# Crowsinc/LiveVisionKit

Hardware: AMD Instinct MI355X
Metric: stabilized frames/sec (one 4K YUV420 stream per GPU, steady state) (higher is better)
Workload: dtype f32

## Files before the change

### include/lvk_hip.h

```cpp
#ifndef LVK_HIP_H
#define LVK_HIP_H

#include <stdint.h>
#include <stddef.h>

#ifdef __cplusplus
extern "C" {
#endif

#define LVK_HIP_OK              0
#define LVK_HIP_ERR_ARG        -1
#define LVK_HIP_ERR_RUNTIME    -2
#define LVK_HIP_ERR_NO_DEVICE  -3

typedef struct lvk_hip_ctx lvk_hip_ctx;


int  lvk_hip_ctx_create(int device, lvk_hip_ctx** out);
int  lvk_hip_ctx_create_on_stream(int device, void* hip_stream, lvk_hip_ctx** out);
void lvk_hip_ctx_destroy(lvk_hip_ctx* ctx);
int  lvk_hip_sync(lvk_hip_ctx* ctx);
void* lvk_hip_stream(lvk_hip_ctx* ctx);
const char* lvk_hip_last_error(lvk_hip_ctx* ctx);
const char* lvk_hip_version(void);
// ... 188 lines not shown
int  lvk_hip_fsr_easu(lvk_hip_ctx* ctx, const void* d_src, int src_step, int rows, int cols, int format, const int region_xywh[4], void* d_dst,
                      int dst_step, int out_rows, int out_cols);
int  lvk_hip_fsr_geometry(int rows, int cols, int out_rows, int out_cols, float multiplier, int maintain_aspect_ratio, const int crop_ltrb[4],
                          int region_xywh[4], int out_rows_cols[2], int* skip);
int  lvk_hip_text_size(const char* text, int scale, int thickness, int wh[2], int* baseline);



int  lvk_hip_stab_prefetch(lvk_hip_stab* stab, const void* d_frame, int step, int rows, int cols, int format);
int  lvk_hip_stab_prefetch_yuv420(lvk_hip_stab* stab, const void* d_y, int y_step, const void* d_u, int u_step, const void* d_v, int v_step,
                                  int nv12, int rows, int cols);
long long lvk_hip_stab_lookahead_frames(lvk_hip_stab* stab);

#define LVK_SCHED_PUSH_FREE_RUNNING   0
#define LVK_SCHED_PUSH_SYNCHRONISED   1
#define LVK_SCHED_INGEST_ON_TRACKER   2
#define LVK_SCHED_INGEST_ON_BULK      3
#define LVK_SCHED_INGEST_INLINE       4
#define LVK_SCHED_REMAP_PERSISTENT    5
#define LVK_SCHED_REMAP_FULL          6
#define LVK_SCHED_WAIT_SIGNAL_WORD    7
#define LVK_SCHED_WAIT_EVENT          8
#define LVK_SCHED_WAIT_WORD_TIMEOUT   9
#define LVK_SCHED_COUNT              10
int  lvk_hip_stab_schedule_counters(lvk_hip_stab* stab, long long out[LVK_SCHED_COUNT], int reset);

int  lvk_hip_stab_get_stats(const lvk_hip_stab* stab, lvk_stab_stats* out);
int  lvk_hip_stab_detector_frames(const lvk_hip_stab* stab, long long* on_device, long long* on_host);
int  lvk_hip_stab_get_meshes(const lvk_hip_stab* stab, float* motion, float* correction, int cap_floats);
int  lvk_hip_stab_get_features(const lvk_hip_stab* stab, float* xy_resp_age, int cap);


#define LVK_STAGE_DOWNSCALE 0
#define LVK_STAGE_PYRAMID   1
#define LVK_STAGE_FAST      2
#define LVK_STAGE_PYRLK     3
#define LVK_STAGE_MOTION    4
#define LVK_STAGE_REMAP     5
#define LVK_STAGE_INGEST    6
#define LVK_STAGE_EGRESS    7
#define LVK_STAGE_COUNT     8
int  lvk_hip_stab_set_profiling(lvk_hip_stab* stab, int enable);
int  lvk_hip_stab_get_profile(lvk_hip_stab* stab, double total_ms[LVK_STAGE_COUNT], long long launches[LVK_STAGE_COUNT]);

int lvk_hip_native_rcp(lvk_hip_ctx* ctx, const float* d_in, float* d_out, size_t n);

typedef struct lvk_hip_mesh_solver lvk_hip_mesh_solver;
// ... 64 lines not shown
```

### livevisionkit_amd/csrc/ingest.hip

```cpp
#include "lvk_hip_internal.hpp"

#include <cmath>
#include <algorithm>
#include <string>

#define LVK_STREAM_STORE(ptr, v) __builtin_nontemporal_store((uint32_t)(v), (ptr))

namespace {

__device__ __forceinline__ uint32_t lin8(const uint8_t* __restrict__ r0, const uint8_t* __restrict__ r1, int pix,
                                         const Lin8Entry tx, int b0, int b1)
{
    const int h0 = r0[tx.s0 * pix] * tx.a0 + r0[tx.s1 * pix] * tx.a1;
    const int h1 = r1[tx.s0 * pix] * tx.a0 + r1[tx.s1 * pix] * tx.a1;
    return (uint32_t)((((b0 * (h0 >> 4)) >> 16) + ((b1 * (h1 >> 4)) >> 16) + 2) >> 2) & 0xffu;
}

template <bool NV12>
__global__ __launch_bounds__(256)
void k_ingest_yuv420(const uint8_t* __restrict__ yp, int y_step, const uint8_t* __restrict__ up, int u_step,
                     const uint8_t* __restrict__ vp, int v_step, int rows, int cols,
                     uint8_t* __restrict__ dst, int dst_step, const Lin8Entry* __restrict__ xtab, const Lin8Entry* __restrict__ ytab, int fast)
{
    const int x0 = (blockIdx.x * 64 + threadIdx.x) * 4;
// ... 9 lines not shown
#pragma unroll
    for (int p = 0; p < 4; p++)
    {
        px[p] = 0;
        if (p < npx)
        {
            const Lin8Entry tx = xtab[x0 + p];
            px[p] = (uint32_t)yp[(long)y * y_step + x0 + p] | (lin8(u0, u1, PIX, tx, ty.a0, ty.a1) << 8) | (lin8(v0, v1, PIX, tx, ty.a0, ty.a1) << 16);
        }
    }
    uint8_t* drow = dst + (long)y * dst_step;
    if (fast && npx == 4)
    {
        uint32_t* d = reinterpret_cast<uint32_t*>(drow + 3 * x0);
        d[0] = px[0] | (px[1] << 24);
        d[1] = (px[1] >> 8) | (px[2] << 16);
        d[2] = (px[2] >> 16) | (px[3] << 8);
    }
    else
        for (int p = 0; p < npx; p++) { uint8_t* d = drow + 3 * (x0 + p); d[0] = (uint8_t)px[p]; d[1] = (uint8_t)(px[p] >> 8); d[2] = (uint8_t)(px[p] >> 16); }
}

template <bool NV12>
__global__ __launch_bounds__(256)
void k_ingest_yuv420_x2(const uint8_t* __restrict__ yp, int y_step, const uint8_t* __restrict__ up, int u_step,
                        const uint8_t* __restrict__ vp, int v_step, int rows, int cols, uint8_t* __restrict__ dst, int dst_step)
{
    LVK_TL(0);
    const int x0 = (blockIdx.x * 64 + threadIdx.x) * 4;
    const int k = blockIdx.y * 4 + threadIdx.y;
    const int cc = cols >> 1, cr = rows >> 1;
    if (x0 >= cols || k > cr) return;
    const int r0 = max(k - 1, 0), r1 = min(k, cr - 1);
    const int c0 = x0 >> 1;
    const bool left = x0 == 0, right = x0 == cols - 4;
    const int lc = left ? 0 : (right ? cc - 4 : c0 - 1);
    struct __attribute__((packed, aligned(1))) P4 { uint32_t w; };
    struct __attribute__((packed, aligned(1))) P8 { uint32_t w[2]; };
    uint32_t su0, su1, sv0, sv1;
    if (NV12)
    {
        const P8 a = *reinterpret_cast<const P8*>(up + (long)r0 * u_step + 2 * lc);
        const P8 b = *reinterpret_cast<const P8*>(up + (long)r1 * u_step + 2 * lc);
        su0 = __builtin_amdgcn_perm(a.w[1], a.w[0], 0x06040200u); sv0 = __builtin_amdgcn_perm(a.w[1], a.w[0], 0x07050301u);
        su1 = __builtin_amdgcn_perm(b.w[1], b.w[0], 0x06040200u); sv1 = __builtin_amdgcn_perm(b.w[1], b.w[0], 0x07050301u);
    }
    else
    {
        su0 = reinterpret_cast<const P4*>(up + (long)r0 * u_step + lc)->w;
        su1 = reinterpret_cast<const P4*>(up + (long)r1 * u_step + lc)->w;
        sv0 = reinterpret_cast<const P4*>(vp + (long)r0 * v_step + lc)->w;
// ... 12 lines not shown
    const int ya = 2 * k - 1, yb = 2 * k;
    const bool has_a = ya >= 0, has_b = yb < rows;
    const uint32_t ywa = has_a ? *reinterpret_cast<const uint32_t*>(yp + (long)ya * y_step + x0) : 0u;
    const uint32_t ywb = has_b ? *reinterpret_cast<const uint32_t*>(yp + (long)yb * y_step + x0) : 0u;
    uint32_t pa[4], pb[4];
#pragma unroll
    for (int p = 0; p < 4; p++)
    {
        const uint32_t u0 = tu0[p], u1 = tu1[p], v0 = tv0[p], v1 = tv1[p];
        const uint32_t ua = ((((u0 + u0 + u0) >> 2) + (u1 >> 2) + 2u) >> 2), ub = (((u0 >> 2) + ((u1 + u1 + u1) >> 2) + 2u) >> 2);
        const uint32_t va = ((((v0 + v0 + v0) >> 2) + (v1 >> 2) + 2u) >> 2), vb = (((v0 >> 2) + ((v1 + v1 + v1) >> 2) + 2u) >> 2);
        pa[p] = ((ywa >> (8 * p)) & 0xffu) | (ua << 8) | (va << 16);
        pb[p] = ((ywb >> (8 * p)) & 0xffu) | (ub << 8) | (vb << 16);
    }
    if (has_a)
    {
        uint32_t* d = reinterpret_cast<uint32_t*>(dst + (long)ya * dst_step + 3 * x0);
        LVK_STREAM_STORE(d + 0, pa[0] | (pa[1] << 24)); LVK_STREAM_STORE(d + 1, (pa[1] >> 8) | (pa[2] << 16)); LVK_STREAM_STORE(d + 2, (pa[2] >> 16) | (pa[3] << 8));
    }
    if (has_b)
    {
        uint32_t* d = reinterpret_cast<uint32_t*>(dst + (long)yb * dst_step + 3 * x0);
        LVK_STREAM_STORE(d + 0, pb[0] | (pb[1] << 24)); LVK_STREAM_STORE(d + 1, (pb[1] >> 8) | (pb[2] << 16)); LVK_STREAM_STORE(d + 2, (pb[2] >> 16) | (pb[3] << 8));
    }
}

template <bool NV12>
__global__ __launch_bounds__(256)
void k_egress_yuv420(const uint8_t* __restrict__ src, int src_step, int rows, int cols,
                     uint8_t* __restrict__ yp, int y_step, uint8_t* __restrict__ up, int u_step, uint8_t* __restrict__ vp, int v_step)
{
    const int cx = blockIdx.x * 64 + threadIdx.x;
    const int cy = blockIdx.y * 4 + threadIdx.y;
    if (cx >= cols / 2 || cy >= rows / 2) return;
    const uint8_t* p0 = src + (long)(2 * cy) * src_step + 6 * (long)cx;
    const uint8_t* p1 = p0 + src_step;
    uint8_t a[6], b[6];
#pragma unroll
    for (int i = 0; i < 6; i++) { a[i] = p0[i]; b[i] = p1[i]; }
    uint8_t* y0 = yp + (long)(2 * cy) * y_step + 2 * cx;
    y0[0] = a[0]; y0[1] = a[3]; y0[y_step] = b[0]; y0[y_step + 1] = b[3];
    const uint8_t u = (uint8_t)((a[1] + a[4] + b[1] + b[4] + 2) >> 2);
    const uint8_t v = (uint8_t)((a[2] + a[5] + b[2] + b[5] + 2) >> 2);
    if (NV12) { uint8_t* d = up + (long)cy * u_step + 2 * cx; d[0] = u; d[1] = v; }
    else { up[(long)cy * u_step + cx] = u; vp[(long)cy * v_step + cx] = v; }
}
// ... 271 lines not shown
        {
            e.s0 = std::min(std::max(s, 0), ssize - 1); e.s1 = std::min(std::max(s + 1, 0), ssize - 1);
            e.a0 = (int)lrintf((1.f - f) * 2048.f); e.a1 = (int)lrintf(f * 2048.f);
        }
        else
        {
            if (s < 0) { f = 0.f; s = 0; }
            bool single = false;
            if (s + 1 >= ssize) { single = true; if (s >= ssize - 1) { f = 0.f; s = ssize - 1; } }
            e.s0 = s; e.s1 = single ? s : s + 1;
            e.a0 = single ? 2048 : (int)lrintf((1.f - f) * 2048.f); e.a1 = single ? 0 : (int)lrintf(f * 2048.f);
        }
        tab[(size_t)d] = e;
    }
    Lin8Entry* d_tab = nullptr;
    LVK_HIP_CHECK(ctx, hipMalloc((void**)&d_tab, tab.size() * sizeof(Lin8Entry)));
    LVK_HIP_CHECK(ctx, hipMemcpy(d_tab, tab.data(), tab.size() * sizeof(Lin8Entry), hipMemcpyHostToDevice));
    ctx->lin8tabs[key] = d_tab;
    *d_out = d_tab;
    return LVK_HIP_OK;
}

int lvk_launch_ingest_yuv420(lvk_hip_ctx* ctx, hipStream_t stream, const void* d_y, int y_step, const void* d_u, int u_step,
                             const void* d_v, int v_step, int nv12, int rows, int cols, void* d_dst, int dst_step)
{
    LVK_HIP_REQUIRE(ctx, d_y && d_u && (nv12 || d_v) && d_dst && rows > 0 && cols > 0);
    LVK_HIP_REQUIRE(ctx, (rows & 1) == 0 && (cols & 1) == 0);
    LVK_HIP_REQUIRE(ctx, y_step >= cols && dst_step >= 3 * cols && u_step >= (nv12 ? cols : cols / 2));
    const Lin8Entry *xt, *yt;
    int rc;
    if ((rc = lvk_get_lin8tab(ctx, cols / 2, cols, false, &xt)) != LVK_HIP_OK) return rc;
    if ((rc = lvk_get_lin8tab(ctx, rows / 2, rows, true, &yt)) != LVK_HIP_OK) return rc;
    const int fast = ((reinterpret_cast<uintptr_t>(d_dst) | (uintptr_t)dst_step) & 3u) == 0 ? 1 : 0;
    const dim3 block(64, 4), grid1((cols / 4 + 63 + (cols % 4 ? 1 : 0)) / 64, (rows + 3) / 4);
    const bool x2 = fast && cols % 4 == 0 && cols >= 16 && rows >= 4 &&
                    ((reinterpret_cast<uintptr_t>(d_y) | (uintptr_t)y_step) & 3u) == 0;
    if (x2)
    {
        const dim3 grid(grid1.x, (rows / 2 + 1 + 3) / 4);
        if (nv12) hipLaunchKernelGGL(k_ingest_yuv420_x2<true>, grid, block, 0, stream, (const uint8_t*)d_y, y_step, (const uint8_t*)d_u, u_step,
                                     (const uint8_t*)d_u, u_step, rows, cols, (uint8_t*)d_dst, dst_step);
        else hipLaunchKernelGGL(k_ingest_yuv420_x2<false>, grid, block, 0, stream, (const uint8_t*)d_y, y_step, (const uint8_t*)d_u, u_step,
                                (const uint8_t*)d_v, v_step, rows, cols, (uint8_t*)d_dst, dst_step);
        LVK_HIP_CHECK(ctx, hipGetLastError());
        return LVK_HIP_OK;
    }
    const dim3 grid = grid1;
    if (nv12)
        hipLaunchKernelGGL(k_ingest_yuv420<true>, grid, block, 0, stream, (const uint8_t*)d_y, y_step, (const uint8_t*)d_u, u_step, (const uint8_t*)d_u, u_step,
                           rows, cols, (uint8_t*)d_dst, dst_step, xt, yt, fast);
    else
        hipLaunchKernelGGL(k_ingest_yuv420<false>, grid, block, 0, stream, (const uint8_t*)d_y, y_step, (const uint8_t*)d_u, u_step, (const uint8_t*)d_v, v_step,
                           rows, cols, (uint8_t*)d_dst, dst_step, xt, yt, fast);
    LVK_HIP_CHECK(ctx, hipGetLastError());
    return LVK_HIP_OK;
}

int lvk_launch_egress_yuv420(lvk_hip_ctx* ctx, hipStream_t stream, const void* d_src, int src_step, int rows, int cols,
                             void* d_y, int y_step, void* d_u, int u_step, void* d_v, int v_step, int nv12)
{
    LVK_HIP_REQUIRE(ctx, d_src && d_y && d_u && (nv12 || d_v) && rows > 0 && cols > 0);
    LVK_HIP_REQUIRE(ctx, (rows & 1) == 0 && (cols & 1) == 0);
    LVK_HIP_REQUIRE(ctx, src_step >= 3 * cols && y_step >= cols && u_step >= (nv12 ? cols : cols / 2));
    const dim3 block(64, 4), grid((cols / 2 + 63) / 64, (rows / 2 + 3) / 4);
    if (nv12)
        hipLaunchKernelGGL(k_egress_yuv420<true>, grid, block, 0, stream, (const uint8_t*)d_src, src_step, rows, cols, (uint8_t*)d_y, y_step, (uint8_t*)d_u, u_step, (uint8_t*)d_u, u_step);
    else
// ... 23 lines not shown
        LVK_HIP_REQUIRE(ctx, (cols & 1) == 0 && steps[0] >= 2 * cols);
        return LVK_HIP_OK;
    case LVK_VIDEO_FORMAT_I444: case LVK_VIDEO_FORMAT_YUVA:
        LVK_HIP_REQUIRE(ctx, p1 && p2 && steps[0] >= cols && steps[1] >= cols && steps[2] >= cols);
        return LVK_HIP_OK;
    case LVK_VIDEO_FORMAT_AYUV:
        LVK_HIP_REQUIRE(ctx, steps[0] >= 4 * cols);
        return LVK_HIP_OK;
    case LVK_VIDEO_FORMAT_Y800:
        LVK_HIP_REQUIRE(ctx, steps[0] >= cols);
        return LVK_HIP_OK;
    case LVK_VIDEO_FORMAT_BGR3:
        LVK_HIP_REQUIRE(ctx, steps[0] >= 3 * cols);
        return LVK_HIP_OK;
    case LVK_VIDEO_FORMAT_RGBA: case LVK_VIDEO_FORMAT_BGRA: case LVK_VIDEO_FORMAT_BGRX:
        LVK_HIP_REQUIRE(ctx, steps[0] == 4 * cols);
        return LVK_HIP_OK;
    default:
        return ctx->fail(LVK_HIP_ERR_ARG, "lvk_hip_ingest_obs: video format " + std::to_string(video_format) + " is not one FrameIngest::Select knows");
    }
}

int lvk_launch_ingest_obs(lvk_hip_ctx* ctx, hipStream_t stream, int video_format, const void* const d_planes[3], const int steps[3],
                          int rows, int cols, void* d_dst, int dst_step)
{
    { const int rc = lvk_ingest_obs_check(ctx, video_format, d_planes, steps, rows, cols); if (rc != LVK_HIP_OK) return rc; }
    LVK_HIP_REQUIRE(ctx, d_dst && dst_step >= (video_format == LVK_VIDEO_FORMAT_Y800 ? cols : 3 * cols));
    const uint8_t* p0 = (const uint8_t*)d_planes[0]; const uint8_t* p1 = (const uint8_t*)d_planes[1]; const uint8_t* p2 = (const uint8_t*)d_planes[2];
    const int fast = ((reinterpret_cast<uintptr_t>(d_dst) | (uintptr_t)dst_step) & 3u) == 0 ? 1 : 0;
    const dim3 block(64, 4), grid((cols + 255) / 256, (rows + 3) / 4);
    switch (video_format)
    {
    case LVK_VIDEO_FORMAT_I420: case LVK_VIDEO_FORMAT_I40A:
        return lvk_launch_ingest_yuv420(ctx, stream, p0, steps[0], p1, steps[1], p2, steps[2], 0, rows, cols, d_dst, dst_step);
    case LVK_VIDEO_FORMAT_NV12:
        return lvk_launch_ingest_yuv420(ctx, stream, p0, steps[0], p1, steps[1], nullptr, 0, 1, rows, cols, d_dst, dst_step);
    case LVK_VIDEO_FORMAT_I422: case LVK_VIDEO_FORMAT_I42A:
        if (fast && cols % 4 == 0 && cols >= 8 && aligned_to(p0, steps[0], 4))
            hipLaunchKernelGGL(k_ingest_422_dw<0>, grid, block, 0, stream, p0, steps[0], p1, steps[1], p2, steps[2], rows, cols, (uint8_t*)d_dst, dst_step);
        else
            hipLaunchKernelGGL(k_ingest_422<0>, grid, block, 0, stream, p0, steps[0], p1, steps[1], p2, steps[2], rows, cols, (uint8_t*)d_dst, dst_step, fast);
        break;
    case LVK_VIDEO_FORMAT_YUY2: case LVK_VIDEO_FORMAT_YVYU: case LVK_VIDEO_FORMAT_UYVY:
        if (fast && cols % 4 == 0 && aligned_to(p0, steps[0], 4))
        {
            if (video_format == LVK_VIDEO_FORMAT_YUY2) hipLaunchKernelGGL(k_ingest_422_dw<1>, grid, block, 0, stream, p0, steps[0], p0, 0, p0, 0, rows, cols, (uint8_t*)d_dst, dst_step);
            else if (video_format == LVK_VIDEO_FORMAT_YVYU) hipLaunchKernelGGL(k_ingest_422_dw<2>, grid, block, 0, stream, p0, steps[0], p0, 0, p0, 0, rows, cols, (uint8_t*)d_dst, dst_step);
            else hipLaunchKernelGGL(k_ingest_422_dw<3>, grid, block, 0, stream, p0, steps[0], p0, 0, p0, 0, rows, cols, (uint8_t*)d_dst, dst_step);
        }
        else if (video_format == LVK_VIDEO_FORMAT_YUY2) hipLaunchKernelGGL(k_ingest_422<1>, grid, block, 0, stream, p0, steps[0], p0, 0, p0, 0, rows, cols, (uint8_t*)d_dst, dst_step, fast);
        else if (video_format == LVK_VIDEO_FORMAT_YVYU) hipLaunchKernelGGL(k_ingest_422<2>, grid, block, 0, stream, p0, steps[0], p0, 0, p0, 0, rows, cols, (uint8_t*)d_dst, dst_step, fast);
        else hipLaunchKernelGGL(k_ingest_422<3>, grid, block, 0, stream, p0, steps[0], p0, 0, p0, 0, rows, cols, (uint8_t*)d_dst, dst_step, fast);
        break;
    case LVK_VIDEO_FORMAT_I444: case LVK_VIDEO_FORMAT_YUVA:
        if (fast && cols % 4 == 0 && aligned_to(p0, steps[0], 4) && aligned_to(p1, steps[1], 4) && aligned_to(p2, steps[2], 4))
            hipLaunchKernelGGL(k_ingest_444_dw<0>, grid, block, 0, stream, p0, steps[0], p1, steps[1], p2, steps[2], rows, cols, (uint8_t*)d_dst, dst_step);
        else
            hipLaunchKernelGGL(k_ingest_444<0>, grid, block, 0, stream, p0, steps[0], p1, steps[1], p2, steps[2], rows, cols, (uint8_t*)d_dst, dst_step, fast);
        break;
// ... 137 lines not shown
```

### livevisionkit_amd/csrc/lvk_hip_internal.hpp

```cpp
#pragma once

#include <hip/hip_runtime.h>
#include <cstdint>
#include <cstdio>
#include <string>
#include <vector>
#include <functional>
#include <map>
#include <set>
#include <mutex>
#include <utility>

#include "lvk_hip.h"

struct LinTabEntry { int s0, s1; float a0, a1; };
struct Lin8Entry { int s0, s1, a0, a1; };
struct AreaTabEntry { int si; float alpha; };
struct FastRegion { int x, y, w, h, threshold, active; };
constexpr int LVK_FAST_INLINE_REGIONS = 8;

constexpr int LVK_MAX_PYR_LEVELS = 8;
struct PyrLevel { const uint8_t* img; const short2* deriv; int rows, cols, step; };
struct PyrArgs { PyrLevel lv[LVK_MAX_PYR_LEVELS]; int nlevels; };

// ... 216 lines not shown
    float2* d_pts = nullptr; float2* d_matched = nullptr; uint8_t* d_status = nullptr;
    float2* d_und = nullptr;
    float2* d_p1 = nullptr; float2* d_p2 = nullptr; int* d_count = nullptr;
    int* h_count = nullptr; float2* h_matched = nullptr; uint8_t* h_status = nullptr;
    int region_w = 0, region_h = 0; double threshold = 0.0;
    bool separate_compact = false;
    bool estimate = true;
    void* d_ws = nullptr; double* h_H = nullptr; int* h_ninl = nullptr; uint8_t* h_mask = nullptr;
    LvkHostSignal done{nullptr, 0};
    void (*stage_boundary)(void* user) = nullptr; void* user = nullptr;
};
int lvk_launch_track_chain(lvk_hip_ctx* ctx, const LvkTrackChain& c);

struct LensArgs;
int lvk_launch_remap_homography(lvk_hip_ctx* ctx, hipStream_t stream, const void* d_src, int src_step, int src_rows, int src_cols,
                                void* d_dst, int dst_step, int dst_rows, int dst_cols, int off_x, int off_y,
                                const float H[9], const uint8_t bg[3], int yuv, const LensArgs* lens = nullptr, bool co_scheduled = false);
int lvk_launch_remap_mesh(lvk_hip_ctx* ctx, hipStream_t stream, const void* d_src, int src_step, int src_rows, int src_cols,
                          void* d_dst, int dst_step, const float* mesh, int mesh_rows, int mesh_cols, const uint8_t bg[3], int yuv,
                          const LensArgs* lens = nullptr, bool co_scheduled = false);
int lvk_launch_warpmesh_apply(lvk_hip_ctx* ctx, hipStream_t stream, const void* d_src, int src_step, int rows, int cols,
                              void* d_dst, int dst_step, const float* mesh, int mesh_rows, int mesh_cols, const uint8_t bg[3], int yuv);

int lvk_launch_ingest_yuv420(lvk_hip_ctx* ctx, hipStream_t stream, const void* d_y, int y_step, const void* d_u, int u_step,
                             const void* d_v, int v_step, int nv12, int rows, int cols, void* d_dst, int dst_step);
int lvk_launch_egress_yuv420(lvk_hip_ctx* ctx, hipStream_t stream, const void* d_src, int src_step, int rows, int cols,
                             void* d_y, int y_step, void* d_u, int u_step, void* d_v, int v_step, int nv12);
int lvk_ingest_obs_check(lvk_hip_ctx* ctx, int video_format, const void* const d_planes[3], const int steps[3], int rows, int cols);
int lvk_launch_ingest_obs(lvk_hip_ctx* ctx, hipStream_t stream, int video_format, const void* const d_planes[3], const int steps[3],
                          int rows, int cols, void* d_dst, int dst_step);
int lvk_launch_egress_obs(lvk_hip_ctx* ctx, hipStream_t stream, int video_format, const void* d_src, int src_step, int rows, int cols,
                          void* const d_planes[3], const int steps[3]);


int lvk_launch_remap_map(lvk_hip_ctx* ctx, hipStream_t stream, const void* d_src, int src_step, int rows, int cols,
                         void* d_dst, int dst_step, const void* d_map, int map_step, const uint8_t bg[3], int yuv);

struct LensModel { double d[17]; float f[17]; int view[4]; };
struct LensModelD { double d[17]; };
__device__ __forceinline__ float2 lvk_lens_undistort_point(const LensModelD& M, double sx, double sy, float2 p)
{
    const double nfx = M.d[0], nfy = M.d[1], ncx = M.d[2], ncy = M.d[3], fx = M.d[4], fy = M.d[5], cx = M.d[6], cy = M.d[7];
    const double k1 = M.d[8], k2 = M.d[9], p1 = M.d[10], p2 = M.d[11], k3 = M.d[12];
    const double kxc = M.d[13], vxc = M.d[14], kyc = M.d[15], vyc = M.d[16];
    const double s = (double)p.x * sx, t = (double)p.y * sy;
    double u = s, v = t;
    for (int pass = 0; pass < 2; pass++)
    {
        const double s1 = s - (u * kxc + vxc), t1 = t - (v * kyc + vyc);
        const double x0 = (s1 - cx) / fx, y0 = (t1 - cy) / fy;
        double x = x0, y = y0;
        for (int j = 0; j < 5; j++)
        {
// ... 49 lines not shown
```

### livevisionkit_amd/csrc/stab_configure.hip

```cpp
#include "stab_state.hpp"

using namespace lvkstab;

int lvk_hip_stab::prof_begin(int kind, hipStream_t stream)
{
    if (!stream) stream = ctx->stream;
    if (!profiling || !((prof_mask >> kind) & 1u) || (prof_tick % prof_every) != 0) return -1;
    if (ev_used >= 1024 && prof_collect() != LVK_HIP_OK) return -1;
    if (ev_used == ev_pool.size())
    {
        EvPair p{nullptr, nullptr, kind};
        if (hipEventCreate(&p.a) != hipSuccess || hipEventCreate(&p.b) != hipSuccess) return -1;
        ev_pool.push_back(p);
    }
    ev_pool[ev_used].kind = kind;
    (void)hipEventRecord(ev_pool[ev_used].a, stream);
    return (int)ev_used++;
}

void lvk_hip_stab::prof_end(int idx, hipStream_t stream) { if (idx >= 0) (void)hipEventRecord(ev_pool[(size_t)idx].b, stream ? stream : ctx->stream); }

int lvk_hip_stab::prof_collect()
{
    LVK_HIP_CHECK(ctx, hipStreamSynchronize(ctx->stream));
// ... 260 lines not shown
                     st->host_trace_acc[0] / st->host_trace_n, st->host_trace_acc[1] / st->host_trace_n, st->host_trace_acc[2] / st->host_trace_n,
                     st->host_trace_acc[3] / st->host_trace_n, st->host_trace_acc[4] / st->host_trace_n);
    st->free_tracker_buffers();
    lvk_mesh_solver_free(st->mesh_dev);
    if (st->h_offsets) (void)hipHostFree(st->h_offsets);
    if (st->h_mesh_status) (void)hipHostFree(st->h_mesh_status);
    st->pyr[0].release(); st->pyr[1].release();
    st->free_pool();
    st->free_hostio();
    if (st->remap_stream)
    {
        (void)hipStreamSynchronize(st->remap_stream);
        rehome_stage_events(st->ctx);
        auto& aux = st->ctx->aux_streams;
        { std::lock_guard<std::mutex> alock(st->ctx->aux_mutex); aux.erase(std::remove(aux.begin(), aux.end(), st->remap_stream), aux.end()); }
        if (st->remap_stream_owned) (void)hipStreamDestroy(st->remap_stream);
    }
    for (int i = 0; i < 2; i++) if (st->remap_done[i]) (void)hipEventDestroy(st->remap_done[i]);
    if (st->ingest_done) (void)hipEventDestroy(st->ingest_done);
    if (st->chain_done) (void)hipEventDestroy(st->chain_done);
    if (st->caller_ready) (void)hipEventDestroy(st->caller_ready);
    if (st->ahead_read_done) (void)hipEventDestroy(st->ahead_read_done);
    if (st->h_chain_flag) (void)hipHostFree(st->h_chain_flag);
    for (auto& p : st->ev_pool) { (void)hipEventDestroy(p.a); (void)hipEventDestroy(p.b); }
    delete st;
}

void* lvk_hip_stab_output_stream(lvk_hip_stab* st)
{
    if (!st) return nullptr;
    return (void*)((st->overlap && st->s.stabilize_output && st->remap_stream) ? st->remap_stream : st->ctx->stream);
}

static void rehome_stage_events(lvk_hip_ctx* ctx)
{
    for (int i = 0; i < lvk_hip_ctx::kStageSlots; i++) if (ctx->stage_done[i]) (void)hipEventRecord(ctx->stage_done[i], ctx->stream);
}

static int stab_detach_bulk_stream(lvk_hip_stab* st)
{
    lvk_hip_ctx* ctx = st->ctx;
    if (!st->remap_stream) return LVK_HIP_OK;
    (void)hipStreamSynchronize(st->remap_stream);
    rehome_stage_events(ctx);
    std::fill(st->slot_read_armed.begin(), st->slot_read_armed.end(), (char)0);
    for (int i = 0; i < 2; i++) if (st->remap_done[i]) (void)hipEventRecord(st->remap_done[i], ctx->stream);
// ... 226 lines not shown
```

### livevisionkit_amd/csrc/stab_state.hpp

```cpp
#pragma once
#include "lvk_hip_internal.hpp"
#include "host_logic.hpp"

#include <chrono>
#include <cstdio>
#include <cstdlib>
#include <cstring>
#include <deque>
#include <functional>
#include <thread>

namespace lvkstab {

using lvkh::Feature;
using lvkh::WarpMeshF;

constexpr int LK_WIN = 11, LK_LEVELS = 3, LK_ITERS = 5;
constexpr double LK_EPS = 0.01, LK_MIN_EIG = 1e-4;
constexpr float HOMOGRAPHY_DISTRIBUTION_THRESHOLD = 0.6f;
constexpr float QA_UPDATE_RATE = 0.1f, QA_BLEND_STEP = 0.05f;

inline void lvk_cpu_relax()
{
#if defined(__x86_64__) || defined(__i386__)
// ... 128 lines not shown
        return true;
    }
    float tracking_stability = 0.0f, scene_quality = 0.0f, trust = 0.0f;
    float last_distribution = 0.0f; int last_detected = 0, last_matched = 0;
    double last_H[9] = {1, 0, 0, 0, 1, 0, 0, 0, 1};
    WarpMeshF last_motion, last_correction;

    bool overlap = false;
    hipStream_t remap_stream = nullptr;
    bool remap_stream_owned = false;
    hipEvent_t remap_done[2] = {nullptr, nullptr};
    int remap_slot = 0;
    const void* pending_release = nullptr;
    bool pool_frames = false;
    int queue_kind = 0;
    std::function<int()> deferred_ingest;
    int run_deferred_ingest() { auto f = std::move(deferred_ingest); deferred_ingest = nullptr; return f ? f() : LVK_HIP_OK; }
    hipEvent_t ingest_done = nullptr;
    unsigned long long ingest_recorded_for = 0;
    hipEvent_t chain_done = nullptr;
    unsigned* h_chain_flag = nullptr; unsigned chain_seq = 0;
    long signal_spin_us = [] { const char* e = std::getenv("LVK_HIP_SIGNAL_SPIN_US"); return e ? std::max(0L, std::atol(e)) : 400L; }();
    bool signal_test_lose = [] { const char* e = std::getenv("LVK_HIP_SIGNAL_TEST_LOSE"); return e && e[0] == '1'; }();
    bool ingest_on_tracker = false, tracker_ingest_capable = false;
    bool bulk_busy_at_push = false;
    bool caller_runs_free = false;
    int assume_caller = [] { const char* e = std::getenv("LVK_HIP_ASSUME_CALLER"); return !e ? 0 : (e[0] == 'f' ? 1 : (e[0] == 's' ? 2 : 0)); }();
    int free_streak = 0, sync_streak = 0;
    std::chrono::steady_clock::time_point last_push_end{};
    long long sched[LVK_SCHED_COUNT] = {0};
    int ingest_placement = [] { const char* e = std::getenv("LVK_HIP_INGEST_PLACEMENT"); return !e ? 0 : (e[0] == 't' ? 1 : (e[0] == 'b' ? 2 : 0)); }();
    std::vector<hipEvent_t> slot_read_done;
    std::vector<char> slot_read_armed;
    int slot_index(const void* p) const { for (size_t i = 0; i < pool_all.size(); i++) if (pool_all[i] == p) return (int)i; return -1; }
    int pending_slot = -1;
    hipEvent_t caller_ready = nullptr;
    bool caller_wait_pending = false;
    int mark_caller_work()
    {
        if (!(overlap && s.stabilize_output && remap_stream)) return LVK_HIP_OK;
        if (hipStreamQuery(ctx->stream) == hipSuccess) { caller_wait_pending = false; return LVK_HIP_OK; }
        (void)hipGetLastError();
        if (!caller_ready) LVK_HIP_CHECK(ctx, hipEventCreateWithFlags(&caller_ready, hipEventDisableTiming));
        LVK_HIP_CHECK(ctx, hipEventRecord(caller_ready, ctx->stream));
        caller_wait_pending = true;
        return LVK_HIP_OK;
// ... 143 lines not shown
```

### livevisionkit_amd/csrc/stabilizer.hip

```cpp
#include "stab_state.hpp"

using namespace lvkstab;

int lvk_hip_stab::track(const QueuedFrame& f, const void* luma, int luma_step, int luma_pix, int luma_channel, WarpMeshF& motion, bool& have_motion)
{
    have_motion = false;
    tracking_stability = 0.0f;
    last_detected = last_matched = 0; last_distribution = 0.0f;
    hipStream_t st = ctx->stream;
    int rc;

    cur ^= 1;
    std::swap(prev_w, cur_w); std::swap(prev_h, cur_h);
    cur_w = s.detection_width; cur_h = s.detection_height;
    DevicePyramid& C = pyr[cur];
    DevicePyramid& P = pyr[cur ^ 1];
    int pe = 0;
    const bool built_ahead = ahead_built_for == push_seq && ahead_built.same(luma, luma_step, luma_pix, luma_channel, f.rows, f.cols) && pyr_w == cur_w && pyr_h == cur_h;
    ahead_built = LumaAhead(); ahead_built_for = 0;
    if (built_ahead) lookahead_frames++;
    else
    {
        pe = prof_begin(LVK_STAGE_DOWNSCALE);
        if ((rc = lvk_launch_luma_area_resize(ctx, luma, luma_step, luma_pix, luma_channel, f.rows, f.cols, const_cast<uint8_t*>(C.args.lv[0].img), C.args.lv[0].step, cur_h, cur_w)) != LVK_HIP_OK) return rc;
// ... 630 lines not shown
        {
            bool used = (p == st->pending_release);
            for (const QueuedFrame& q : st->queue) used = used || (q.d_ptr == p);
            if (!used) st->pool_free.push_back(p);
        }
        LVK_HIP_REQUIRE(ctx, !st->pool_free.empty());
    }
    void* slot = st->pool_free.front(); st->pool_free.pop_front();
    const bool side_ingest = st->overlap && st->s.stabilize_output && !direct;
    st->tracker_ingest_capable = side_ingest && st->queue_capacity > 1;
    st->ingest_on_tracker = false;
    int pe = 0;
    auto do_ingest = [=]() -> int {
        const bool on_tracker = side_ingest && st->ingest_on_tracker;
        st->sched[on_tracker ? LVK_SCHED_INGEST_ON_TRACKER : (side_ingest ? LVK_SCHED_INGEST_ON_BULK : LVK_SCHED_INGEST_INLINE)]++;
        hipStream_t is = (side_ingest && !on_tracker) ? st->remap_stream : ctx->stream;
        if (side_ingest && !on_tracker) { const int w = st->bulk_stream_sees_caller_work(); if (w != LVK_HIP_OK) return w; }
        if (on_tracker)
        {
            const int si = st->slot_index(slot);
            if (si >= 0 && st->slot_read_armed[(size_t)si]) { st->slot_read_armed[(size_t)si] = 0; LVK_HIP_CHECK(ctx, hipStreamWaitEvent(is, st->slot_read_done[(size_t)si], 0)); }
        }
        for (hipEvent_t& e : st->ingest_wait) if (e) { LVK_HIP_CHECK(ctx, hipStreamWaitEvent(is, e, 0)); e = nullptr; }
        const int pi = st->prof_begin(LVK_STAGE_INGEST, is);
        const int r = lvk_launch_ingest_obs(ctx, is, vf, ip.data(), is_.data(), rows, cols, slot, 3 * cols);
        st->prof_end(pi, is);
        if (r != LVK_HIP_OK) return r;
        if (side_ingest)
        {
            if (!st->ingest_done) LVK_HIP_CHECK(ctx, hipEventCreateWithFlags(&st->ingest_done, hipEventDisableTiming));
            LVK_HIP_CHECK(ctx, hipEventRecord(st->ingest_done, is));
            st->ingest_recorded_for = st->push_seq;
        }
        return LVK_HIP_OK;
    };
    if (side_ingest) st->deferred_ingest = do_ingest;
    else { rc = do_ingest(); if (rc != LVK_HIP_OK) { const int r1 = st->return_slot(slot); return r1 != LVK_HIP_OK ? r1 : rc; } }
    int prod = 0; const void* released = nullptr;
    st->pool_frames = side_ingest;
    OutPlanes420 o420{o_y, oy_step, o_u, ou_step, o_v, ov_step, nv12, false, o_rows};
    if (!(o_y && o_u && (nv12 || o_v))) o420.y = nullptr;
    const bool fused_obs = !is420 && lvk_remap_obs_fusable(vf) && op[0];
    if (fused_obs) { o420.vf = vf; o420.y = op[0]; for (int i = 0; i < 3; i++) { o420.p[i] = op[i]; o420.s[i] = os[i]; } }
    lvk_frame_info info{0, 0, 0};
    {
        QueuedFrame due{};
        const bool will = st->next_output(QueuedFrame{slot, 3 * cols, rows, cols, timestamp, frame_format}, &due);
        const int out_cols = will ? due.cols : cols;
        rc = lvk_stab_push_impl(st, slot, 3 * cols, rows, cols, timestamp, frame_format, direct ? slot : (const void*)luma, direct ? 3 * cols : luma_step, direct ? 3 : luma_pix,
                                st->pool_out, 3 * out_cols, (int)(st->pool_out_bytes / ((size_t)3 * out_cols)), &prod, out_timestamp, &released,
                                (is420 || fused_obs) ? &o420 : nullptr, &info);
    }
    {
        bool taken = released == slot;
        for (const QueuedFrame& q : st->queue) taken = taken || q.d_ptr == slot;
        if (!taken) { st->deferred_ingest = nullptr; const int r1 = st->return_slot(slot, true); if (rc == LVK_HIP_OK) rc = r1; }
    }
    if (st->deferred_ingest) { const int r2 = st->run_deferred_ingest(); if (rc == LVK_HIP_OK) rc = r2; }
    if (released)
    {
        if (st->is_retired(released)) { const int r3 = st->release_retired(released); if (rc == LVK_HIP_OK) rc = r3; }
        else { const int r3 = st->return_slot(const_cast<void*>(released)); if (rc == LVK_HIP_OK) rc = r3; }
    }
    if (emitted && prod) *emitted = info;
    if (side_ingest)
    {
        if (st->ahead_built_for == st->push_seq + 1) st->finish_post();
        st->trace.mark(HostTrace::EXIT_PRE);
        if (st->ingest_recorded_for == st->push_seq) LVK_HIP_CHECK(ctx, hipEventSynchronize(st->ingest_done));
        st->trace.mark(HostTrace::EXIT_WAIT);
    }
    else if (!st->s.stabilize_output || direct) LVK_HIP_CHECK(ctx, hipStreamSynchronize(ctx->stream));
    if (rc != LVK_HIP_OK) return rc;
    if (prod && o420.used) { if (produced) *produced = 1; }
    else if (prod)
    {
        if (is420)
        {
            LVK_HIP_REQUIRE(ctx, o_y && o_u && (nv12 || o_v));
            LVK_HIP_REQUIRE(ctx, oy_step >= info.cols && ou_step >= (nv12 ? info.cols : info.cols / 2) && (nv12 || ov_step >= info.cols / 2) && o_rows >= info.rows);
        }
        else LVK_HIP_REQUIRE(ctx, op[0] && o_rows >= info.rows);
        hipStream_t es = (st->overlap && st->s.stabilize_output) ? st->remap_stream : ctx->stream;
        if (st->remap_wait) { const hipEvent_t e = st->remap_wait; st->remap_wait = nullptr; LVK_HIP_CHECK(ctx, hipStreamWaitEvent(es, e, 0)); }
        pe = st->prof_begin(LVK_STAGE_EGRESS, es);
        rc = lvk_launch_egress_obs(ctx, es, vf, st->pool_out, 3 * info.cols, info.rows, info.cols, op.data(), os.data());
        st->prof_end(pe, es);
        if (rc != LVK_HIP_OK) return rc;
        if (produced) *produced = 1;
    }
    st->trace.mark(HostTrace::EXIT);
    st->last_push_end = std::chrono::steady_clock::now();
// ... 22 lines not shown
```

### livevisionkit_amd/stabilization.py

```python
import ctypes
import time

import numpy as np

from . import _native
from .context import Context

_c = ctypes

FORMAT_BGR, FORMAT_BGRA, FORMAT_RGB, FORMAT_RGBA, FORMAT_YUV, FORMAT_GRAY = range(6)
CHANNELS = {FORMAT_BGR: 3, FORMAT_BGRA: 4, FORMAT_RGB: 3, FORMAT_RGBA: 4, FORMAT_YUV: 3, FORMAT_GRAY: 1}


def frame_args(frame, channels, kind="uint8"):
    if (frame.dim() != 3 or frame.shape[2] != channels or frame.stride(2) != 1 or frame.stride(1) != channels
            or frame.dtype.itemsize != 1):
        raise ValueError("a packed %s frame [rows, cols, %d] with contiguous rows is required" % (kind, channels))
    return frame.data_ptr(), frame.stride(0)


def out_frame(out, frame, shape, message):
    if out is None:
        import torch
        return torch.empty(shape, dtype=torch.uint8, device=frame.device)
# ... 320 lines not shown

    def ready(self):
        return bool(self.lib.lvk_hip_stab_ready(self.handle))

    def frame_delay(self):
        return int(self.lib.lvk_hip_stab_frame_delay(self.handle))

    def stable_region(self, rows, cols):
        r = (_c.c_int * 4)()
        self.ctx._check(self.lib.lvk_hip_stab_stable_region(self.handle, rows, cols, r))
        return tuple(r)

    def stats(self):
        st = StabStats()
        self.ctx._check(self.lib.lvk_hip_stab_get_stats(self.handle, _c.byref(st)))
        return st

    def detector_frames(self):
        a = _c.c_longlong(0); b = _c.c_longlong(0)
        self.ctx._check(self.lib.lvk_hip_stab_detector_frames(self.handle, _c.byref(a), _c.byref(b)))
        return a.value, b.value

    SCHEDULE = ("push_free_running", "push_synchronised", "ingest_on_tracker", "ingest_on_bulk", "ingest_inline", "remap_persistent", "remap_full",
                "wait_signal_word", "wait_event", "wait_word_timeout")

    def schedule_counters(self, reset=False):
        a = (_c.c_longlong * len(self.SCHEDULE))()
        self.ctx._check(self.lib.lvk_hip_stab_schedule_counters(self.handle, a, 1 if reset else 0))
        return {k: int(a[i]) for i, k in enumerate(self.SCHEDULE)}

    def meshes(self):
        n = self._settings.motion_width * self._settings.motion_height * 2
        a = np.zeros(n, np.float32); b = np.zeros(n, np.float32)
        self.lib.lvk_hip_stab_get_meshes(self.handle, a.ctypes.data_as(_c.POINTER(_c.c_float)), b.ctypes.data_as(_c.POINTER(_c.c_float)), n)
        shp = (self._settings.motion_height, self._settings.motion_width, 2)
        return a.reshape(shp), b.reshape(shp)

    def features(self, cap=8192):
        a = np.zeros((cap, 4), np.float32)
        n = self.lib.lvk_hip_stab_get_features(self.handle, a.ctypes.data_as(_c.POINTER(_c.c_float)), cap)
        return a[:max(n, 0)].copy()

    def draw_trackers(self):
        self.ctx._check(self.lib.lvk_hip_stab_draw_trackers(self.handle))

    def draw_motion_mesh(self):
        self.ctx._check(self.lib.lvk_hip_stab_draw_motion_mesh(self.handle))
# ... 50 lines not shown
```

Before: 8740.

## Signal ingest completion via host-visible word instead of event synchronize

The YUV420 x2 ingest kernel now counts finished blocks with device atomics in per-row and global tickets. The last block writes a sequence number to a coherent host-pinned word. On the free-running tracker path, the host spins on that word for up to a fixed budget instead of calling hipEventSynchronize on ingest_done, falling back to the event on timeout. This aims to cut event-wait latency on the push path, at the cost of extra atomics, a __syncthreads per block and host CPU spinning.

```diff
diff --git a/include/lvk_hip.h b/include/lvk_hip.h
--- a/include/lvk_hip.h
+++ b/include/lvk_hip.h
@@ -234,7 +234,10 @@
 #define LVK_SCHED_WAIT_SIGNAL_WORD    7
 #define LVK_SCHED_WAIT_EVENT          8
 #define LVK_SCHED_WAIT_WORD_TIMEOUT   9
-#define LVK_SCHED_COUNT              10
+#define LVK_SCHED_CONV_WAIT_WORD   10
+#define LVK_SCHED_CONV_WAIT_EVENT  11
+#define LVK_SCHED_CONV_WAIT_WORD_TIMEOUT 12
+#define LVK_SCHED_COUNT              13
 int  lvk_hip_stab_schedule_counters(lvk_hip_stab* stab, long long out[LVK_SCHED_COUNT], int reset);
 
 int  lvk_hip_stab_get_stats(const lvk_hip_stab* stab, lvk_stab_stats* out);
diff --git a/livevisionkit_amd/csrc/ingest.hip b/livevisionkit_amd/csrc/ingest.hip
--- a/livevisionkit_amd/csrc/ingest.hip
+++ b/livevisionkit_amd/csrc/ingest.hip
@@ -55,11 +55,10 @@
 }
 
 template <bool NV12>
-__global__ __launch_bounds__(256)
-void k_ingest_yuv420_x2(const uint8_t* __restrict__ yp, int y_step, const uint8_t* __restrict__ up, int u_step,
-                        const uint8_t* __restrict__ vp, int v_step, int rows, int cols, uint8_t* __restrict__ dst, int dst_step)
-{
-    LVK_TL(0);
+__device__ __forceinline__
+void ingest_yuv420_x2_thread(const uint8_t* __restrict__ yp, int y_step, const uint8_t* __restrict__ up, int u_step,
+                             const uint8_t* __restrict__ vp, int v_step, int rows, int cols, uint8_t* __restrict__ dst, int dst_step)
+{
     const int x0 = (blockIdx.x * 64 + threadIdx.x) * 4;
     const int k = blockIdx.y * 4 + threadIdx.y;
     const int cc = cols >> 1, cr = rows >> 1;
@@ -118,6 +117,23 @@
     {
         uint32_t* d = reinterpret_cast<uint32_t*>(dst + (long)yb * dst_step + 3 * x0);
         LVK_STREAM_STORE(d + 0, pb[0] | (pb[1] << 24)); LVK_STREAM_STORE(d + 1, (pb[1] >> 8) | (pb[2] << 16)); LVK_STREAM_STORE(d + 2, (pb[2] >> 16) | (pb[3] << 8));
+    }
+}
+
+template <bool NV12>
+__global__ __launch_bounds__(256)
+void k_ingest_yuv420_x2(const uint8_t* __restrict__ yp, int y_step, const uint8_t* __restrict__ up, int u_step,
+                        const uint8_t* __restrict__ vp, int v_step, int rows, int cols, uint8_t* __restrict__ dst, int dst_step, LvkPlanesRead read)
+{
+    LVK_TL(0);
+    ingest_yuv420_x2_thread<NV12>(yp, y_step, up, u_step, vp, v_step, rows, cols, dst, dst_step);
+    if (read.flag)
+    {
+        __syncthreads();
+        if (threadIdx.x == 0 && threadIdx.y == 0 &&
+            __hip_atomic_fetch_add(read.tickets + 1 + blockIdx.y, 1u, __ATOMIC_RELAXED, __HIP_MEMORY_SCOPE_AGENT) + 1u == read.row_target &&
+            __hip_atomic_fetch_add(read.tickets, 1u, __ATOMIC_RELAXED, __HIP_MEMORY_SCOPE_AGENT) + 1u == read.target)
+            __hip_atomic_store(read.flag, read.seq, __ATOMIC_RELAXED, __HIP_MEMORY_SCOPE_SYSTEM);
     }
 }
 
@@ -435,8 +451,10 @@
 }
 
 int lvk_launch_ingest_yuv420(lvk_hip_ctx* ctx, hipStream_t stream, const void* d_y, int y_step, const void* d_u, int u_step,
-                             const void* d_v, int v_step, int nv12, int rows, int cols, void* d_dst, int dst_step)
-{
+                             const void* d_v, int v_step, int nv12, int rows, int cols, void* d_dst, int dst_step, LvkPlanesRead* read)
+{
+    LvkPlanesRead rd{};
+    if (read) { rd = *read; read->flag = nullptr; }
     LVK_HIP_REQUIRE(ctx, d_y && d_u && (nv12 || d_v) && d_dst && rows > 0 && cols > 0);
     LVK_HIP_REQUIRE(ctx, (rows & 1) == 0 && (cols & 1) == 0);
     LVK_HIP_REQUIRE(ctx, y_step >= cols && dst_step >= 3 * cols && u_step >= (nv12 ? cols : cols / 2));
@@ -451,11 +469,14 @@
     if (x2)
     {
         const dim3 grid(grid1.x, (rows / 2 + 1 + 3) / 4);
+        if (rd.flag && rd.tickets && grid.y <= rd.rows_cap) { rd.row_target += grid.x; rd.target += grid.y; }
+        else rd = LvkPlanesRead{};
         if (nv12) hipLaunchKernelGGL(k_ingest_yuv420_x2<true>, grid, block, 0, stream, (const uint8_t*)d_y, y_step, (const uint8_t*)d_u, u_step,
-                                     (const uint8_t*)d_u, u_step, rows, cols, (uint8_t*)d_dst, dst_step);
+                                     (const uint8_t*)d_u, u_step, rows, cols, (uint8_t*)d_dst, dst_step, rd);
         else hipLaunchKernelGGL(k_ingest_yuv420_x2<false>, grid, block, 0, stream, (const uint8_t*)d_y, y_step, (const uint8_t*)d_u, u_step,
-                                (const uint8_t*)d_v, v_step, rows, cols, (uint8_t*)d_dst, dst_step);
+                                (const uint8_t*)d_v, v_step, rows, cols, (uint8_t*)d_dst, dst_step, rd);
         LVK_HIP_CHECK(ctx, hipGetLastError());
+        if (read) *read = rd;
         return LVK_HIP_OK;
     }
     const dim3 grid = grid1;
@@ -525,8 +546,10 @@
 }
 
 int lvk_launch_ingest_obs(lvk_hip_ctx* ctx, hipStream_t stream, int video_format, const void* const d_planes[3], const int steps[3],
-                          int rows, int cols, void* d_dst, int dst_step)
-{
+                          int rows, int cols, void* d_dst, int dst_step, LvkPlanesRead* read)
+{
+    const bool is420 = video_format == LVK_VIDEO_FORMAT_I420 || video_format == LVK_VIDEO_FORMAT_I40A || video_format == LVK_VIDEO_FORMAT_NV12;
+    if (read && !is420) read->flag = nullptr;
     { const int rc = lvk_ingest_obs_check(ctx, video_format, d_planes, steps, rows, cols); if (rc != LVK_HIP_OK) return rc; }
     LVK_HIP_REQUIRE(ctx, d_dst && dst_step >= (video_format == LVK_VIDEO_FORMAT_Y800 ? cols : 3 * cols));
     const uint8_t* p0 = (const uint8_t*)d_planes[0]; const uint8_t* p1 = (const uint8_t*)d_planes[1]; const uint8_t* p2 = (const uint8_t*)d_planes[2];
@@ -535,9 +558,9 @@
     switch (video_format)
     {
     case LVK_VIDEO_FORMAT_I420: case LVK_VIDEO_FORMAT_I40A:
-        return lvk_launch_ingest_yuv420(ctx, stream, p0, steps[0], p1, steps[1], p2, steps[2], 0, rows, cols, d_dst, dst_step);
+        return lvk_launch_ingest_yuv420(ctx, stream, p0, steps[0], p1, steps[1], p2, steps[2], 0, rows, cols, d_dst, dst_step, read);
     case LVK_VIDEO_FORMAT_NV12:
-        return lvk_launch_ingest_yuv420(ctx, stream, p0, steps[0], p1, steps[1], nullptr, 0, 1, rows, cols, d_dst, dst_step);
+        return lvk_launch_ingest_yuv420(ctx, stream, p0, steps[0], p1, steps[1], nullptr, 0, 1, rows, cols, d_dst, dst_step, read);
     case LVK_VIDEO_FORMAT_I422: case LVK_VIDEO_FORMAT_I42A:
         if (fast && cols % 4 == 0 && cols >= 8 && aligned_to(p0, steps[0], 4))
             hipLaunchKernelGGL(k_ingest_422_dw<0>, grid, block, 0, stream, p0, steps[0], p1, steps[1], p2, steps[2], rows, cols, (uint8_t*)d_dst, dst_step);
diff --git a/livevisionkit_amd/csrc/lvk_hip_internal.hpp b/livevisionkit_amd/csrc/lvk_hip_internal.hpp
--- a/livevisionkit_amd/csrc/lvk_hip_internal.hpp
+++ b/livevisionkit_amd/csrc/lvk_hip_internal.hpp
@@ -262,13 +262,15 @@
 int lvk_launch_warpmesh_apply(lvk_hip_ctx* ctx, hipStream_t stream, const void* d_src, int src_step, int rows, int cols,
                               void* d_dst, int dst_step, const float* mesh, int mesh_rows, int mesh_cols, const uint8_t bg[3], int yuv);
 
+struct LvkPlanesRead { unsigned* tickets = nullptr; unsigned rows_cap = 0, row_target = 0, target = 0; unsigned* flag = nullptr; unsigned seq = 0; };
+
 int lvk_launch_ingest_yuv420(lvk_hip_ctx* ctx, hipStream_t stream, const void* d_y, int y_step, const void* d_u, int u_step,
-                             const void* d_v, int v_step, int nv12, int rows, int cols, void* d_dst, int dst_step);
+                             const void* d_v, int v_step, int nv12, int rows, int cols, void* d_dst, int dst_step, LvkPlanesRead* read = nullptr);
 int lvk_launch_egress_yuv420(lvk_hip_ctx* ctx, hipStream_t stream, const void* d_src, int src_step, int rows, int cols,
                              void* d_y, int y_step, void* d_u, int u_step, void* d_v, int v_step, int nv12);
 int lvk_ingest_obs_check(lvk_hip_ctx* ctx, int video_format, const void* const d_planes[3], const int steps[3], int rows, int cols);
 int lvk_launch_ingest_obs(lvk_hip_ctx* ctx, hipStream_t stream, int video_format, const void* const d_planes[3], const int steps[3],
-                          int rows, int cols, void* d_dst, int dst_step);
+                          int rows, int cols, void* d_dst, int dst_step, LvkPlanesRead* read = nullptr);
 int lvk_launch_egress_obs(lvk_hip_ctx* ctx, hipStream_t stream, int video_format, const void* d_src, int src_step, int rows, int cols,
                           void* const d_planes[3], const int steps[3]);
 
diff --git a/livevisionkit_amd/csrc/stab_configure.hip b/livevisionkit_amd/csrc/stab_configure.hip
--- a/livevisionkit_amd/csrc/stab_configure.hip
+++ b/livevisionkit_amd/csrc/stab_configure.hip
@@ -306,6 +306,8 @@
     if (st->caller_ready) (void)hipEventDestroy(st->caller_ready);
     if (st->ahead_read_done) (void)hipEventDestroy(st->ahead_read_done);
     if (st->h_chain_flag) (void)hipHostFree(st->h_chain_flag);
+    if (st->h_conv_flag) (void)hipHostFree(st->h_conv_flag);
+    if (st->d_conv_tickets) (void)hipFree(st->d_conv_tickets);
     for (auto& p : st->ev_pool) { (void)hipEventDestroy(p.a); (void)hipEventDestroy(p.b); }
     delete st;
 }
diff --git a/livevisionkit_amd/csrc/stab_state.hpp b/livevisionkit_amd/csrc/stab_state.hpp
--- a/livevisionkit_amd/csrc/stab_state.hpp
+++ b/livevisionkit_amd/csrc/stab_state.hpp
@@ -174,6 +174,12 @@
     unsigned* h_chain_flag = nullptr; unsigned chain_seq = 0;
     long signal_spin_us = [] { const char* e = std::getenv("LVK_HIP_SIGNAL_SPIN_US"); return e ? std::max(0L, std::atol(e)) : 400L; }();
     bool signal_test_lose = [] { const char* e = std::getenv("LVK_HIP_SIGNAL_TEST_LOSE"); return e && e[0] == '1'; }();
+    static constexpr long CONV_SPIN_US = 5000;
+    static constexpr unsigned CONV_TICKET_ROWS = 2048;
+    unsigned* h_conv_flag = nullptr; unsigned* d_conv_tickets = nullptr;
+    unsigned conv_seq = 0, conv_row_total = 0, conv_ticket_total = 0;
+    int conv_rows = 0, conv_cols = 0;
+    bool conv_word_armed = false;
     bool ingest_on_tracker = false, tracker_ingest_capable = false;
     bool bulk_busy_at_push = false;
     bool caller_runs_free = false;
diff --git a/livevisionkit_amd/csrc/stabilizer.hip b/livevisionkit_amd/csrc/stabilizer.hip
--- a/livevisionkit_amd/csrc/stabilizer.hip
+++ b/livevisionkit_amd/csrc/stabilizer.hip
@@ -676,10 +676,27 @@
             if (si >= 0 && st->slot_read_armed[(size_t)si]) { st->slot_read_armed[(size_t)si] = 0; LVK_HIP_CHECK(ctx, hipStreamWaitEvent(is, st->slot_read_done[(size_t)si], 0)); }
         }
         for (hipEvent_t& e : st->ingest_wait) if (e) { LVK_HIP_CHECK(ctx, hipStreamWaitEvent(is, e, 0)); e = nullptr; }
+        LvkPlanesRead read{};
+        st->conv_word_armed = false;
+        if (on_tracker && st->caller_runs_free)
+        {
+            const size_t ticket_bytes = (1 + (size_t)lvk_hip_stab::CONV_TICKET_ROWS) * sizeof(unsigned);
+            if (!st->h_conv_flag) { LVK_HIP_CHECK(ctx, hipHostMalloc((void**)&st->h_conv_flag, 64, hipHostMallocCoherent)); *st->h_conv_flag = 0; }
+            if (!st->d_conv_tickets) { LVK_HIP_CHECK(ctx, hipMalloc((void**)&st->d_conv_tickets, ticket_bytes)); st->conv_rows = st->conv_cols = 0; }
+            if (rows != st->conv_rows || cols != st->conv_cols)
+            {
+                LVK_HIP_CHECK(ctx, hipMemsetAsync(st->d_conv_tickets, 0, ticket_bytes, is));
+                st->conv_row_total = st->conv_ticket_total = 0; st->conv_rows = rows; st->conv_cols = cols;
+            }
+            read.tickets = st->d_conv_tickets; read.rows_cap = lvk_hip_stab::CONV_TICKET_ROWS;
+            read.row_target = st->conv_row_total; read.target = st->conv_ticket_total;
+            read.flag = st->h_conv_flag; read.seq = st->conv_seq + 1;
+        }
         const int pi = st->prof_begin(LVK_STAGE_INGEST, is);
-        const int r = lvk_launch_ingest_obs(ctx, is, vf, ip.data(), is_.data(), rows, cols, slot, 3 * cols);
+        const int r = lvk_launch_ingest_obs(ctx, is, vf, ip.data(), is_.data(), rows, cols, slot, 3 * cols, read.flag ? &read : nullptr);
         st->prof_end(pi, is);
         if (r != LVK_HIP_OK) return r;
+        if (read.flag) { st->conv_seq = read.seq; st->conv_row_total = read.row_target; st->conv_ticket_total = read.target; st->conv_word_armed = true; }
         if (side_ingest)
         {
             if (!st->ingest_done) LVK_HIP_CHECK(ctx, hipEventCreateWithFlags(&st->ingest_done, hipEventDisableTiming));
@@ -721,7 +738,25 @@
     {
         if (st->ahead_built_for == st->push_seq + 1) st->finish_post();
         st->trace.mark(HostTrace::EXIT_PRE);
-        if (st->ingest_recorded_for == st->push_seq) LVK_HIP_CHECK(ctx, hipEventSynchronize(st->ingest_done));
+        if (st->ingest_recorded_for == st->push_seq)
+        {
+            bool planes_read = false;
+            if (st->conv_word_armed)
+            {
+                const unsigned expect = st->signal_test_lose ? st->conv_seq + 0x40000000u : st->conv_seq;
+                const auto t0 = std::chrono::steady_clock::now();
+                const auto budget = std::chrono::microseconds(lvk_hip_stab::CONV_SPIN_US);
+                for (unsigned spins = 0;; spins++)
+                {
+                    if (__atomic_load_n(st->h_conv_flag, __ATOMIC_ACQUIRE) == expect) { planes_read = true; break; }
+                    if ((spins & 63u) == 63u && std::chrono::steady_clock::now() - t0 > budget) break;
+                    lvk_cpu_relax();
+                }
+                st->sched[planes_read ? LVK_SCHED_CONV_WAIT_WORD : LVK_SCHED_CONV_WAIT_WORD_TIMEOUT]++;
+            }
+            if (!planes_read) { LVK_HIP_CHECK(ctx, hipEventSynchronize(st->ingest_done)); st->sched[LVK_SCHED_CONV_WAIT_EVENT]++; }
+        }
+        st->conv_word_armed = false;
         st->trace.mark(HostTrace::EXIT_WAIT);
     }
     else if (!st->s.stabilize_output || direct) LVK_HIP_CHECK(ctx, hipStreamSynchronize(ctx->stream));
diff --git a/livevisionkit_amd/stabilization.py b/livevisionkit_amd/stabilization.py
--- a/livevisionkit_amd/stabilization.py
+++ b/livevisionkit_amd/stabilization.py
@@ -366,7 +366,7 @@
         return a.value, b.value
 
     SCHEDULE = ("push_free_running", "push_synchronised", "ingest_on_tracker", "ingest_on_bulk", "ingest_inline", "remap_persistent", "remap_full",
-                "wait_signal_word", "wait_event", "wait_word_timeout")
+                "wait_signal_word", "wait_event", "wait_word_timeout", "conv_wait_word", "conv_wait_event", "conv_wait_word_timeout")
 
     def schedule_counters(self, reset=False):
         a = (_c.c_longlong * len(self.SCHEDULE))()
```

Measured after the change: 8154. 6.7% lower.
